# dvl-tum/e-osvos

Hardware: AMD Instinct MI355X
Metric: finetune_iters_per_sec (higher is better)
Workload: dtype f32 (f16x3 split); 1 GPU; e-OSVOS-50 fine-tune iteration (BASELINE configs[1]): DeepLabV3+-ResNet50, batch 3, 480x854, BCE, per-neuron-lr SGD; one (sequence, object) per rank; batch=3, height=480, width=854, parallelism=replicas x1

## Files before the change

### e-osvos_amd/_ffi.py

```python
import ctypes
import os

_HERE = os.path.dirname(os.path.abspath(__file__))
LIB_PATH = os.environ.get('EOSVOS_LIB') or os.path.join(_HERE, 'libeosvos.so')

c_float_p = ctypes.c_void_p
_E = ctypes.c_void_p

_SIGNATURES = {
    'eosvos_version': (ctypes.c_char_p, []),
    'eosvos_last_error': (ctypes.c_char_p, []),
    'eosvos_set_matrix_mode': (ctypes.c_int, [ctypes.c_int]),
    'eosvos_get_matrix_mode': (ctypes.c_int, []),
    'eosvos_set_presplit': (ctypes.c_int, [ctypes.c_int]),
    'eosvos_plan_fingerprint': (ctypes.c_int, [_E, ctypes.POINTER(ctypes.c_uint64)]),
    'eosvos_set_engine_matrix_mode': (ctypes.c_int, [_E, ctypes.c_int]),
    'eosvos_get_engine_matrix_mode': (ctypes.c_int, [_E]),
    'eosvos_set_wg_budget': (ctypes.c_int, [_E, ctypes.c_int]),
    'eosvos_set_side_stream': (ctypes.c_int, [_E, ctypes.c_int]),
    'eosvos_num_convs': (ctypes.c_int, [ctypes.c_int]),
    'eosvos_conv_info': (ctypes.c_int, [ctypes.c_int, ctypes.c_int, ctypes.POINTER(ctypes.c_int64)]),
    'eosvos_param_count': (ctypes.c_int64, [ctypes.c_int]),
    'eosvos_lr_count': (ctypes.c_int64, [ctypes.c_int]),
    'eosvos_norm_count': (ctypes.c_int64, [ctypes.c_int]),
    'eosvos_create': (ctypes.c_int, [ctypes.POINTER(_E), ctypes.c_int, ctypes.c_int, ctypes.c_int,
                                     ctypes.c_int, ctypes.c_int, ctypes.c_int, ctypes.c_void_p]),
    'eosvos_create_ex': (ctypes.c_int, [ctypes.POINTER(_E), ctypes.c_int, ctypes.c_int, ctypes.c_int,
                                        ctypes.c_int, ctypes.c_int, ctypes.c_int, ctypes.c_void_p, ctypes.c_int]),
    'eosvos_destroy': (ctypes.c_int, [_E]),
# ... 123 lines not shown
```

### e-osvos_amd/csrc/conv_kernels.hip

```cpp
#include "kernels.h"

#include <stdlib.h>
#include <string.h>

#include <vector>

namespace eosvos {

typedef float f32x16 __attribute__((ext_vector_type(16)));

#define EOSVOS_BK 32
#define EOSVOS_EB 4
#define EOSVOS_EB128 EOSVOS_EB
#define EOSVOS_OCC 2
#define MFMA32(a, b, c) __builtin_amdgcn_mfma_f32_32x32x2f32((a), (b), (c), 0, 0, 0)

__device__ __forceinline__ int xcd_remap(int bid, int nwg) {
  const int q = nwg >> 3, r = nwg & 7, xcd = bid & 7;
  return (xcd < r ? xcd * (q + 1) : r * (q + 1) + (xcd - r) * q) + (bid >> 3);
}

__device__ __forceinline__ float4 ldg4(const float* p) { return *reinterpret_cast<const float4*>(p); }
__device__ __forceinline__ float4 bufld4(__amdgpu_buffer_rsrc_t r, unsigned byte_off) {
  auto v = __builtin_amdgcn_raw_buffer_load_b128(r, byte_off, 0, 0);
// ... 456 lines not shown
long conv_build_multi_table(const ConvArgs& a, const ConvSegHost* segs, int nseg, std::vector<int>& prefix,
                            std::vector<unsigned char>& taplist, std::vector<ConvTap>& taps) {
  const int chunks = (a.Kc + EOSVOS_BK - 1) / EOSVOS_BK;
  const int nt = (a.N + 127) / 128, mt = (a.M + 127) / 128;
  taps.clear();
  for (int g = 0; g < nseg; ++g) {
    const ConvSegHost& sg = segs[g];
    const int T = sg.k * sg.k;
    for (int ky = 0; ky < sg.k; ++ky)
      for (int kx = 0; kx < sg.k; ++kx) {
        ConvTap t;
        t.dy = sg.pad - ky * sg.dil; t.dx = sg.pad - kx * sg.dil;
        t.xoff = sg.xoff;
        t.wbase = (int)(sg.woff + (long)(ky * sg.k + kx) * a.wK);
        t.wrow = T * a.wK;
        t.ksoff = sg.ksoff; t.seg = g; t.pad_ = 0;
        taps.push_back(t);
      }
  }
  prefix.assign((size_t)mt * nt + 1, 0);
  taplist.assign((size_t)mt * nt * 32, 0);
  long total = 0;
  for (int tm = 0; tm < mt; ++tm) {
    std::vector<unsigned char> keep;
    for (size_t id = 0; id < taps.size(); ++id) {
      bool any = false;
      for (int m = tm * 128; m < a.M && m < tm * 128 + 128 && !any; ++m) {
        const int hw = a.Ho * a.Wo, rem = m % hw;
        const int sy = rem / a.Wo + taps[id].dy, sx = rem % a.Wo + taps[id].dx;
        any = sy >= 0 && sx >= 0 && sy < a.Hi && sx < a.Wi;
      }
// ... 151 lines not shown
            c = MFMA_BF16(fa[tm][0], fb[tn][1], c);
            c = MFMA_BF16(fa[tm][0], fb[tn][0], c);
          } else {
            c = MFMA_F16(__builtin_bit_cast(f16x8, fa[tm][1]), __builtin_bit_cast(f16x8, fb[tn][0]), c);
            c = MFMA_F16(__builtin_bit_cast(f16x8, fa[tm][0]), __builtin_bit_cast(f16x8, fb[tn][1]), c);
            c = MFMA_F16(__builtin_bit_cast(f16x8, fa[tm][0]), __builtin_bit_cast(f16x8, fb[tn][0]), c);
          }
          acc[hm + tm][hn + tn] = c;
        }
    }
  }
}

constexpr int xs_max(int a, int b) { return a > b ? a : b; }
template <int BN, int NP> constexpr int conv_xs_smem() { return xs_max(NP * (128 + BN) * X6_ROWB, 128 * (BN + 4) * 4); }
template <int BN, bool KMAJOR, int NP, bool MULTI = false>
__device__ __forceinline__ void conv_xs_body(const ConvArgs& p, unsigned char* smem) {
  constexpr int BM = 128, BK = 32;
  constexpr int A_BYTES = NP * BM * X6_ROWB;
  constexpr int LDC = BN + 4;
  unsigned char* const As = smem;
  unsigned char* const Bs = smem + A_BYTES;

  const int tid = threadIdx.x, lane = tid & 63, wave = tid >> 6;
  const int wm = wave >> 1, wn = wave & 1;
  const int fr = lane & 15, fq = lane >> 4;

  const int T = p.KH * p.KW;
  const int chunks = (p.Kc + BK - 1) / BK;
  const int ksteps = T * chunks;
  const int nt = (p.N + BN - 1) / BN;
  const int tiles = ((p.M + BM - 1) / BM) * nt;
  const long U = p.tprefix ? (long)p.tprefix[tiles] : (long)tiles * ksteps;
// ... 2 lines not shown
  const long u_begin = sk0 + (long)bid * p.per;
  long u_end = u_begin + p.per;
  if (u_end > U) u_end = U;
  int dp_i = 0;

  constexpr int APASS = BM / 32;
  const int a_c4 = tid & 7, a_r = x6_stage_row(tid);
  constexpr int NQ = BN / 4, RPT = BN / 32;
  constexpr int BPASS = BN / 32;
  const int b_c4 = a_c4, b_r = a_r;
  const int b_n4 = RPT == 4 ? x6_kmaj_c4_128(tid) : x6_kmaj_c4_64(tid);
  const int b_kq = RPT == 4 ? x6_kmaj_kq_128(tid) : x6_kmaj_kq_64(tid);
  const int up = 1 << p.upshift;
  constexpr int TN = BN / 32;
  const __amdgpu_buffer_rsrc_t rx = make_rsrc(p.x, (long)p.B * p.Hi * p.Wi * p.ldx * 4);
  const __amdgpu_buffer_rsrc_t rw = make_rsrc(p.w, MULTI ? p.w_floats * 4 : (p.plane_rows ? (long)p.nplanes : 1L) * p.wN * T * p.wK * 4);
  float sa = 1.f, sb = 1.f, inv_ab = 1.f;
  unsigned h3_ax = 0, h3_ak = 0, h3_aw = 0;
  bool h3_pending = false;
  if (NP == 2 && !MULTI) {
    h3_ax = amax_issue(p.amax_x); h3_ak = amax_issue(KMAJOR ? p.amax_ks : nullptr); h3_aw = amax_issue(p.amax_w);
    h3_pending = true;
  }
  auto scales_late = [&]() {
    if (h3_pending) {
      float ia, ib;
      sa = h3_scale_bits(h3_ax, KMAJOR && p.amax_ks, h3_ak, ia);
      sb = h3_scale_bits(h3_aw, false, 0u, ib);
      inv_ab = ia * ib;
      h3_pending = false;
    }
// ... 81 lines not shown
        a_sx0[i] = ox * p.mul + p.off0;
        a_img[i] = b * p.Hi * p.Wi;
      } else {
        a_sy0[i] = -(1 << 28);
        a_sx0[i] = 0;
        a_img[i] = 0;
      }
    }
    float4 ra[APASS], rb[BPASS];
    constexpr unsigned OOB = 0x80000000u;
    int a_off[APASS];
    int b_off[BPASS];
    const int wplane = p.plane_rows ? (m0 / p.plane_rows) * (int)p.w_plane : 0;
#pragma unroll
    for (int i = 0; i < BPASS; ++i) {
      if (KMAJOR) {
        const int n = n0 + b_n4 * 4;
        b_off[i] = n < p.N ? wplane + (b_kq * RPT + i) * T * p.wK + n : -1;
      } else {
        const int n = n0 + b_r + i * 32;
        b_off[i] = n < p.N ? wplane + n * T * p.wK + b_c4 * 4 : -1;
      }
    }
    int cur_tap = -1;
    int m_wrow = 0, m_ksoff = 0;
    auto load_tiles = [&](int ks) {
      const int vt = ks / chunks;
      const int c0 = (ks - vt * chunks) * BK;
      const int tap = MULTI ? vt : (p.tprefix ? (int)((tappack >> (4 * vt)) & 15) : vt);
      if (tap != cur_tap) {
        cur_tap = tap;
        int dy, dx, xoff = 0;
        if (MULTI) {
          const int id = __builtin_amdgcn_readfirstlane((int)p.taplist[(size_t)tile * 32 + vt]);
          const ConvTap d = p.taps[id];
          dy = d.dy; dx = d.dx; xoff = d.xoff; m_wrow = d.wrow; m_ksoff = d.ksoff; seg_ld = d.seg;
          if (NP == 2) { sa = pick4(seg_sa, seg_ld); sb = pick4(seg_sb, seg_ld); }
#pragma unroll
          for (int i = 0; i < BPASS; ++i) {
            const int n = n0 + b_n4 * 4;
            b_off[i] = n < p.N ? d.wbase + (b_kq * RPT + i) * d.wrow + n : -1;
          }
        } else {
          const int ky = tap / p.KW, kx = tap - ky * p.KW;
          dy = ky * p.kstep; dx = kx * p.kstep;
        }
#pragma unroll
        for (int i = 0; i < APASS; ++i) {
          const int sy = a_sy0[i] + dy, sx = a_sx0[i] + dx;
          bool ok = sy >= 0 && sx >= 0 && ((sy | sx) & (up - 1)) == 0;
          const int iy = sy >> p.upshift, ix = sx >> p.upshift;
          ok = ok && iy < p.Hi && ix < p.Wi;
          a_off[i] = ok ? (a_img[i] + iy * p.Wi + ix) * p.ldx + a_c4 * 4 + xoff : -1;
        }
      }
      const bool cok = (c0 + a_c4 * 4) < p.Kc;
      float4 ks4 = make_float4(1.f, 1.f, 1.f, 1.f);
      if (KMAJOR && p.kscale && cok) ks4 = ldg4(p.kscale + (MULTI ? m_ksoff : 0) + c0 + a_c4 * 4);
#pragma unroll
      for (int i = 0; i < APASS; ++i) {
        const unsigned off = (cok && a_off[i] >= 0) ? (unsigned)(a_off[i] + c0) * 4u : OOB;
        float4 v = bufld4(rx, off);
        if (KMAJOR) { v.x *= ks4.x; v.y *= ks4.y; v.z *= ks4.z; v.w *= ks4.w; }
        ra[i] = v;
      }
#pragma unroll
      for (int i = 0; i < BPASS; ++i) {
        unsigned off;
        if (MULTI) {
          const int k = c0 + b_kq * RPT + i;
          off = (b_off[i] >= 0 && k < p.Kc) ? (unsigned)(b_off[i] + c0 * m_wrow) * 4u : OOB;
        } else if (KMAJOR) {
          const int k = c0 + b_kq * RPT + i;
          off = (b_off[i] >= 0 && k < p.Kc) ? (unsigned)(b_off[i] + (c0 * T + tap) * p.wK) * 4u : OOB;
        } else {
          const int k = c0 + b_c4 * 4;
          off = (b_off[i] >= 0 && k < p.Kc) ? (unsigned)(b_off[i] + tap * p.wK + c0) * 4u : OOB;
        }
        rb[i] = bufld4(rw, off);
      }
    };
    auto store_tiles = [&]() {
#pragma unroll
      for (int i = 0; i < APASS; ++i) {
        uint2 pc[NP];
        xs_split4<NP>(ra[i].x, ra[i].y, ra[i].z, ra[i].w, sa, pc);
#pragma unroll
        for (int q = 0; q < NP; ++q) *reinterpret_cast<uint2*>(As + (q * BM + a_r + i * 32) * X6_ROWB + a_c4 * 8) = pc[q];
      }
      if (!KMAJOR) {
#pragma unroll
        for (int i = 0; i < BPASS; ++i) {
          uint2 pc[NP];
          xs_split4<NP>(rb[i].x, rb[i].y, rb[i].z, rb[i].w, sb, pc);
#pragma unroll
          for (int q = 0; q < NP; ++q) *reinterpret_cast<uint2*>(Bs + (q * BN + b_r + i * 32) * X6_ROWB + b_c4 * 8) = pc[q];
        }
      } else if (RPT == 4) {
#pragma unroll
        for (int j = 0; j < 4; ++j) {
          uint2 pc[NP];
          xs_split4<NP>(f4c(rb[0], j), f4c(rb[1], j), f4c(rb[RPT == 4 ? 2 : 0], j), f4c(rb[RPT == 4 ? 3 : 0], j), sb, pc);
#pragma unroll
          for (int q = 0; q < NP; ++q) *reinterpret_cast<uint2*>(Bs + (q * BN + j * NQ + b_n4) * X6_ROWB + b_kq * 8) = pc[q];
        }
// ... 120 lines not shown
        for (int lr = c_r; lr < BM; lr += CROWS)
          *reinterpret_cast<float4*>(slab + lr * BN + c_c4 * 4) = *reinterpret_cast<const float4*>(Cs + lr * LDC + c_c4 * 4);
      }
    }
    if (!dp) u += ks_end - ks_begin;
  }
  if (NP == 2 && p.amax_y) amax_block_commit(ymax, p.amax_y);
}

template <int BN, bool KMAJOR>
__global__ __launch_bounds__(256, 2) void conv_x6_kernel(const ConvArgs p) {
  __shared__ __attribute__((aligned(16))) unsigned char smem[conv_xs_smem<BN, 3>()];
  conv_xs_body<BN, KMAJOR, 3>(p, smem);
}
#define EOSVOS_H3_OCC64 2
template <int BN, bool KMAJOR>
__global__ __launch_bounds__(256, BN == 64 ? EOSVOS_H3_OCC64 : 2) void conv_h3_kernel(const ConvArgs p) {
  __shared__ __attribute__((aligned(16))) unsigned char smem[conv_xs_smem<BN, 2>()];
  conv_xs_body<BN, KMAJOR, 2>(p, smem);
}
__global__ __launch_bounds__(256, 2) void conv_h3_multi_kernel(const ConvArgs p) {
  __shared__ __attribute__((aligned(16))) unsigned char smem[conv_xs_smem<128, 2>()];
  conv_xs_body<128, true, 2, true>(p, smem);
}
__global__ __launch_bounds__(256, 2) void conv_x6_multi_kernel(const ConvArgs p) {
  __shared__ __attribute__((aligned(16))) unsigned char smem[conv_xs_smem<128, 3>()];
  conv_xs_body<128, true, 3, true>(p, smem);
}

__device__ __forceinline__ void amax_block_commit8(unsigned m, unsigned* slot) {
  __shared__ unsigned wmax8[8];
#pragma unroll
  for (int o = 32; o > 0; o >>= 1) {
    const unsigned t = (unsigned)__shfl_xor((int)m, o);
    m = m > t ? m : t;
  }
  if ((threadIdx.x & 63) == 0) wmax8[threadIdx.x >> 6] = m;
  __syncthreads();
// ... 1031 lines not shown
bool g_prof_on = false;
std::vector<ProfRec> g_prof;
std::vector<hipEvent_t> g_prof_pool;
const char* const kProfNames[] = {
    "conv_x6_kernel<128, false>", "conv_x6_kernel<128, true>", "conv_x6_kernel<64, false>", "conv_x6_kernel<64, true>",
    "wgrad_x6_kernel<128, 128>", "wgrad_x6_kernel<128, 64>", "wgrad_x6_kernel<64, 128>", "wgrad_x6_kernel<64, 64>",
    "conv_igemm_kernel<128, false, *>", "conv_igemm_kernel<128, true, *>", "conv_igemm_kernel<64, false, 0>", "conv_igemm_kernel<64, true, 0>",
    "wgrad_kernel<128, 128>", "wgrad_kernel<128, 64>", "wgrad_kernel<64, 128>", "wgrad_kernel<64, 64>",
    "conv_fixup_kernel",
    "wgrad_x6_group_kernel<128, 128>", "wgrad_x6_group_kernel<128, 64>", "wgrad_x6_group_kernel<64, 128>", "wgrad_x6_group_kernel<64, 64>",
    "conv_h3_kernel<128, false>", "conv_h3_kernel<128, true>", "conv_h3_kernel<64, false>", "conv_h3_kernel<64, true>",
    "wgrad_h3_kernel<128, 128>", "wgrad_h3_kernel<128, 64>", "wgrad_h3_kernel<64, 128>", "wgrad_h3_kernel<64, 64>",
    "wgrad_h3_group_kernel<128, 128>", "wgrad_h3_group_kernel<128, 64>", "wgrad_h3_group_kernel<64, 128>", "wgrad_h3_group_kernel<64, 64>",
    "conv_h3_multi_kernel", "conv_x6_multi_kernel", "conv1x1_stream_kernel<*, 128>", "conv1x1_stream_kernel<*, 64>",
    "conv3x3_stream_kernel",
    "wgrad_p_kernel<256, 256>", "wgrad_p_group_kernel<256, 256>"};
constexpr int kProfKernels = sizeof(kProfNames) / sizeof(kProfNames[0]);
hipEvent_t prof_event() {
  if (!g_prof_pool.empty()) { hipEvent_t e = g_prof_pool.back(); g_prof_pool.pop_back(); return e; }
  hipEvent_t e;
  (void)hipEventCreate(&e);
  return e;
}
struct ProfScope {
  hipStream_t s;
  bool on;
  ProfScope(int kernel, double flops, hipStream_t st) : s(st), on(g_prof_on) {
    if (!on) return;
    ProfRec r{prof_event(), prof_event(), kernel, flops};
    (void)hipEventRecord(r.a, s);
    g_prof.push_back(r);
  }
// ... 109 lines not shown
  {
    constexpr long min_avg = 16, min_chunk = 12, min_fill = 60;
    const bool even_taps = a.total_units <= 0 || a.total_units * 100 >= 85L * tiles * ksteps;
    const long budget = conv_wg_budget(a.wg_budget);
    const long avg = a.total_units > 0 ? a.total_units / tiles : ksteps;
    const long S = tiles > 0 ? budget / tiles : 0;
    if (conv_mfma_mode() == 2 && !a.deep && even_taps && q == 0 && per > 0 && per < avg && S >= 2 && avg >= min_avg && avg / S >= min_chunk &&
        tiles * S * 100 >= min_fill * budget) {
      a.splitk = (int)S; nwg = tiles * S; per = 0;
    }
  }
  a.dp_q = (int)q; a.per = (int)per; a.nwg = (int)nwg;
  return (int)nwg;
}

void launch_conv(ConvArgs& a, hipStream_t s) {
  if (stream3x3_ok(a)) {
    a.dp_q = 0; a.per = 0; a.nwg = 0; a.splitk = 0;
    ProfScope ps(37, 2.0 * a.M * a.N * a.Kc * 9, s);
    launch_stream3x3(a, s);
    return;
  }
  if (const int nc = stream1x1_nc(a)) {
    a.dp_q = 0; a.per = 0; a.nwg = 0; a.splitk = 0;
    ProfScope ps(nc >= 128 ? 35 : 36, 2.0 * a.M * a.N * a.Kc, s);
    if (nc == 128) {
      if (a.Kc == 64) launch_stream1x1<64, 128>(a, s);
      else if (a.Kc == 128) launch_stream1x1<128, 128>(a, s);
      else if (a.Kc == 304) launch_stream1x1<304, 128>(a, s);
      else launch_stream1x1<256, 128>(a, s);
// ... 6 lines not shown
      else if (a.Kc == 304) launch_stream1x1<304, 64>(a, s);
      else launch_stream1x1<512, 64>(a, s);
    }
    return;
  }
  const int bn = conv_bn(a);
  const int nwg = conv_plan(a);
  const long tiles = (long)((a.M + 127) / 128) * ((a.N + bn - 1) / bn);
  const dim3 grid(nwg), block(256);
  const int mode = conv_mfma_mode();
  a.y2_done = (a.y2 && mode == 2) ? 1 : 0;
  const int pk = a.nseg > 0 ? (mode == 2 ? 33 : 34) : (mode == 2 ? 21 : mode == 1 ? 0 : 8) + (bn == 128 ? 0 : 2) + (a.kmajor ? 1 : 0);
  {
  ProfScope ps(pk, 2.0 * a.M * a.N * a.KH * a.KW * a.Kc * conv_exec_frac(a), s);
  if (a.nseg > 0) {
    if (mode == 2) hipLaunchKernelGGL(conv_h3_multi_kernel, grid, block, 0, s, a);
    else hipLaunchKernelGGL(conv_x6_multi_kernel, grid, block, 0, s, a);
  } else if (mode == 2) {
    if (a.kmajor) {
      if (bn == 128) hipLaunchKernelGGL((conv_h3_kernel<128, true>), grid, block, 0, s, a);
      else hipLaunchKernelGGL((conv_h3_kernel<64, true>), grid, block, 0, s, a);
    } else {
      if (bn == 128) hipLaunchKernelGGL((conv_h3_kernel<128, false>), grid, block, 0, s, a);
      else hipLaunchKernelGGL((conv_h3_kernel<64, false>), grid, block, 0, s, a);
    }
  } else if (mode == 1) {
    if (a.kmajor) {
      if (bn == 128) hipLaunchKernelGGL((conv_x6_kernel<128, true>), grid, block, 0, s, a);
      else hipLaunchKernelGGL((conv_x6_kernel<64, true>), grid, block, 0, s, a);
    } else {
      if (bn == 128) hipLaunchKernelGGL((conv_x6_kernel<128, false>), grid, block, 0, s, a);
      else hipLaunchKernelGGL((conv_x6_kernel<64, false>), grid, block, 0, s, a);
    }
  } else if (a.deep == 1) {
    if (a.kmajor) hipLaunchKernelGGL((conv_igemm_kernel<128, true, 1>), grid, block, 0, s, a);
    else hipLaunchKernelGGL((conv_igemm_kernel<128, false, 1>), grid, block, 0, s, a);
// ... 284 lines not shown
```

### e-osvos_amd/csrc/engine.cpp

```cpp
#include <dlfcn.h>
#include <hip/hip_runtime.h>
#include <math.h>
#include <stdio.h>
#include <stdlib.h>
#include <string.h>

#include <algorithm>
#include <cmath>
#include <functional>
#include <map>
#include <set>
#include <string>
#include <vector>

#include "../../include/eosvos.h"
#include "kernels.h"

using namespace eosvos;

static thread_local std::string g_err;
static int fail(const std::string& m) {
  g_err = m;
  return 1;
}
// ... 217 lines not shown
  struct PairBuf {
    unsigned char* p = nullptr;
    float* sc = nullptr;
    int64_t floats = 0;
    bool want = false;
    bool fresh = true;
    bool covered = false;
    long cover_iter = -1;
  };
  std::map<const float*, PairBuf> pairs[2];
  long pair_iter = 0;
  unsigned char* pair_zero = nullptr;
  float* pair_sc_pool = nullptr;
  int pair_sc_used = 0;
  uint64_t plan_fp[2] = {0, 0};
  bool presplit_inflight = false;
  int mode = -1;
  int plan_mode = -1;

  unsigned* amax = nullptr;
  struct AmaxRec { const void* ptr = nullptr; long epoch = -1, zero_epoch = -1; };
  std::vector<AmaxRec> amax_rec;
  long fwd_epoch = 0, bwd_epoch = 0;
  bool w_amax_valid = false;
  long us_zero_epoch = -1;
  long* mt_rbase = nullptr; int* mt_rlen = nullptr; long* mt_toff = nullptr; int2* mt_tit = nullptr; int mt_nent = 0;
  long* amax_w_off = nullptr;
  int* amax_w_n = nullptr;
  std::vector<char> ks_amax_valid;
  struct TRec { int idx; bool valid; };
// ... 31 lines not shown
    allocs.push_back(p);
    return (float*)p;
  }
  float* W_(int ci) { return Wp + t.convs[ci].poff; }
  bool gn() const { return norm_mode == EOSVOS_NORM_GN16; }
  const float* A_(int ci) const { return (t.convs[ci].norm && !gn()) ? na + t.convs[ci].noff : nullptr; }
  const float* G_(int ci) const { return na + t.convs[ci].noff; }
  const float* B_(int ci) const { return t.convs[ci].norm ? nb + t.convs[ci].noff : nullptr; }
};

namespace {

void wino_weights_changed(eosvos_engine* e) {
  for (auto& kv : e->wino_us_valid) kv.second = 0;
  e->w_amax_valid = false;
}

bool trace_on();
enum { AM_X = 0, AM_V = 1, AM_G = 2, AM_DM = 3, AM_W = 4, AM_U = 5, AM_US = 6, AM_KS = 7, AM_KINDS = 8 };
inline size_t amax_col(const eosvos_engine* e, int kind, int ci) {
  const size_t nc = e->t.convs.size(), T = eosvos_engine::TSLOTS;
  if (kind <= AM_V) return (size_t)kind * nc + ci;
  if (kind <= AM_DM) return 2 * nc + T + (size_t)(kind - AM_G) * nc + ci;
  return 4 * nc + 2 * T + (size_t)(kind - AM_W) * nc + ci;
}
inline size_t amax_tcol(const eosvos_engine* e, int phase, int idx) {
  return (phase == 0 ? 2 : 4) * e->t.convs.size() + (size_t)phase * eosvos_engine::TSLOTS + idx;
}
inline void amax_zero(unsigned* first, size_t count, hipStream_t st) { launch_amax_zero(first, (int)count, st); }
inline bool h3_mode() { return conv_mfma_mode() == 2; }
// ... 99 lines not shown
    std::vector<int> n(nc);
    for (size_t ci = 0; ci < nc; ++ci) {
      const ConvL& c = e->t.convs[ci];
      off[ci] = (long)c.poff;
      n[ci] = ((c.cin & 3) || (c.poff & 3)) ? 0 : (int)c.wsize();
    }
    e->amax_w_off = (long*)e->falloc((int64_t)nc * 2);
    e->amax_w_n = (int*)e->falloc((int64_t)nc);
    if (!e->amax_w_off || !e->amax_w_n) return;
    (void)hipMemcpy(e->amax_w_off, off.data(), nc * sizeof(long), hipMemcpyHostToDevice);
    (void)hipMemcpy(e->amax_w_n, n.data(), nc * sizeof(int), hipMemcpyHostToDevice);
  }
  amax_zero(amax_slot(e, AM_W, 0), nc, st);
  launch_absmax_segments(e->Wp, e->amax_w_off, e->amax_w_n, (int)nc, amax_slot(e, AM_W, 0), st);
  e->w_amax_valid = true;
}
const unsigned* amax_ks(eosvos_engine* e, int ci, hipStream_t st) {
  if (amax_init(e) || !e->A_(ci)) return nullptr;
  if (!e->ks_amax_valid[ci]) {
    amax_make(e, AM_KS, ci, e->A_(ci), 1, e->t.convs[ci].cout, e->t.convs[ci].cout, st);
    e->ks_amax_valid[ci] = 1;
  }
  return amax_slot(e, AM_KS, ci);
}
unsigned* amax_wino_weights(eosvos_engine* e, int ci, hipStream_t st) {
  if (!h3_mode() || amax_init(e)) return nullptr;
  unsigned* u = amax_slot(e, AM_U, ci);
  if (e->us_zero_epoch != e->fwd_epoch) {
    amax_zero(u, 1, st);
    amax_zero(amax_slot(e, AM_US, ci), 1, st);
// ... 173 lines not shown
    a.res = res; a.ldres = ldres; a.relu = relu ? 1 : 0;
    if (relu)
      if (uint8_t* m = e->m8w(ykey)) { a.mask8_out = m + (y - ykey) / 4; a.ldm8_out = ldy / 4; }
  }
  attach_tap_table(e, ci, 0, B, a);
  unsigned* gn_yslot = nullptr;
  if (h3_mode() && !amax_init(e)) {
    amax_weights(e, st);
    a.amax_x = tlookup(e, 0, xkey);
    if (!a.amax_x) a.amax_x = amax_get(e, AM_X, ci, x, (long)B * Hi * Wi, c.cin, ldx, st);
    a.amax_w = amax_slot(e, AM_W, ci);
    gn_yslot = twrite_fused(e, 0, ykey, ldy == c.cout);
    if (!gn) a.amax_y = gn_yslot;
  }
  if (!gn && !side) pair_attach(e, 0, ykey, y, ldy == c.cout, a);
  trace("fwd", ci, a.M, a.N, (long)c.T() * c.cin, conv_plan(a), conv_exec_frac(a));
  launch_conv(a, st);
  pair_covered(e, 0, ykey, a);
  if (gn)
    launch_gn_forward(e->zbuf[ci], c.cout, e->G_(ci), e->nb + c.noff, res, ldres, y, ldy, e->gn_stats[ci], e->gn_partial, B,
                      a.Ho * a.Wo, c.cout, 1e-5f, relu ? 1 : 0, st, gn ? gn_yslot : nullptr,
                      (relu && e->m8w(ykey)) ? e->m8w(ykey) + (y - ykey) / 4 : nullptr, ldy / 4);
}
bool dgrad_has_tail(const ConvArgs& a) { return a.N > 128 && a.N % 128 > 0 && a.N % 128 <= 64; }
void launch_dgrad_tail_split(eosvos_engine* e, int ci, ConvArgs a, long K) {
  const int tail = a.N % 128;
  ConvArgs b = a;
  a.N -= tail;
  trace("dgrad", ci, a.M, a.N, K, conv_plan(a));
  launch_conv(a, e->s);
  b.N = tail; b.w += a.N; b.y += a.N;
  if (b.mask8) { b.mask8 += a.N / 4; b.mask_c0 = b.mask_c0 > a.N ? b.mask_c0 - a.N : 0; }
  if (b.res) b.res += a.N;
  trace("dgrad", ci, b.M, b.N, K, conv_plan(b));
  launch_conv(b, e->s);
}
int conv_dgrad(eosvos_engine* e, int ci, const float* g, int ldg, int Hin, int Win, float* gx, int ldgx, int B,
               bool accum, const float* relu_x, int mask_c0, const float* add = nullptr, int ldadd = 0,
               const float* gkey = nullptr, const float* gxkey = nullptr) {
  const uint8_t* mask8 = relu_x ? e->m8(relu_x) : nullptr;
  if (relu_x && !mask8) return fail("internal: a masked data gradient of conv " + std::to_string(ci) + " has no ReLU mask bytes");
  const ConvL& c = e->t.convs[ci];
  ConvArgs a;
// ... 44 lines not shown
    }
    launch_wino_dgrad_output(wg.tm, e->wino_dv, prow, c.cin, B, Hin, Win, th, tw, wg.d, mask8, a.ldm8, mask_c0, accum ? 1 : 0, gx, ldgx, e->s, gxs);
    return 0;
  }
  if (c.k == 1 && c.stride == 2 && !add) {
    if (!accum) (void)hipMemsetAsync(gx, 0, (size_t)B * Hin * Win * ldgx * sizeof(float), e->s);
    a.Ho = a.Hi; a.Wo = a.Wi; a.mul = 1; a.off0 = 0; a.kstep = 0; a.upshift = 0;
    a.M = B * a.Ho * a.Wo; a.dst_up = 1; a.Hf = Hin; a.Wf = Win;
  }
  if (dgrad_has_tail(a) && !a.dst_up && !(c.k == 3 && c.dil >= 2)) {
    launch_dgrad_tail_split(e, ci, a, (long)c.T() * c.cout);
    return 0;
  }
  attach_tap_table(e, ci, 1, B, a);
  pair_attach(e, 1, gxkey, gx, ldgx == c.cin, a);
  trace("dgrad", ci, a.M, a.N, (long)c.T() * c.cout, conv_plan(a), conv_exec_frac(a));
  launch_conv(a, e->s);
  pair_covered(e, 1, gxkey, a);
  return 0;
}
#define EOSVOS_SIDE_BATCH 4
int g_presplit = -1;
bool presplit_switch() {
  if (g_presplit < 0) g_presplit = (getenv("EOSVOS_PRESPLIT") && atoi(getenv("EOSVOS_PRESPLIT")) == 0) ? 0 : 1;
  return g_presplit != 0;
}
bool presplit_enabled(const eosvos_engine* e) {
  return presplit_switch() && h3_mode() && e->force_algo == 0 && (e->s2 || e->presplit_inflight);
}
bool presplit_wgrad_shape(const ConvL& c, int P, int ldg, int ldx) {
// ... 378 lines not shown
  }
  unsigned* amax_w = nullptr;
  if (update) {
    for (auto& kv : e->wino_us_valid)
      if (e->train_from == 0 || kv.first >= lo) kv.second = 0;
    if (h3_mode() && !amax_init(e) && e->w_amax_valid) {
      amax_w = amax_slot(e, AM_W, 0);
      amax_zero(amax_w + lo, (size_t)(hi - lo), stream);
    } else {
      e->w_amax_valid = false;
    }
  }
  launch_sgd_update_all(e->upd_tab[slot], hi - lo, e->upd_blocks[slot], e->Wp, e->ws_wg, e->na,
                        update ? e->lr : nullptr, (update && e->lr_level == EOSVOS_LR_PARAM) ? e->lr_elem : nullptr,
                        accumulate ? e->gsum : nullptr, e->keep_grads ? e->gout : nullptr, stream, amax_w);
  return 0;
}

bool aspp_dgrad_merged(eosvos_engine* e, int B, float* g_l4, const float* l4) {
  const Topo& t = e->t;
  if (e->gn() || !conv_multi_supported() || e->force_algo != 0) return false;
  for (int i = 0; i < 4; ++i) {
    const ConvL& c = t.convs[t.aspp[i]];
    if (c.cout != 256 || c.cin != t.convs[t.aspp[0]].cin || c.stride != 1 || t.aspp[i] != t.aspp[0] + i) return false;
    if (wino_on(e, t.aspp[i], B, e->h16, e->w16)) return false;
  }
  const ConvL& c0 = t.convs[t.aspp[0]];
  ConvArgs a;
  memset(&a, 0, sizeof(a));
  a.wg_budget = e->wg_budget;
// ... 36 lines not shown
    a.amax_x = tlookup(e, 1, e->g_cat);
    if (!a.amax_x) a.amax_x = amax_get(e, AM_G, t.aspp[0], e->g_cat, (long)B * e->h16 * e->w16, 1280, 1280, e->s);
    for (int i = 0; i < 4; ++i) {
      a.seg_amax_w[i] = amax_slot(e, AM_W, t.aspp[i]);
      a.seg_amax_ks[i] = amax_ks(e, t.aspp[i], e->s);
    }
    a.amax_y = twrite_fused(e, 1, g_l4, true);
  }
  double fl = 0;
  for (int i = 0; i < 4; ++i) fl += 2.0 * a.M * a.N * t.convs[t.aspp[i]].T() * 256.0;
  if (trace_on())
    trace_line("dgrad", t.aspp[0], a.M, a.N, (long)(a.total_units * 32 / (((a.M + 127) / 128) * ((a.N + 127) / 128))), conv_plan(a),
               2.0 * 128 * 128 * 32 * (double)a.total_units);
  (void)fl;
  pair_attach(e, 1, g_l4, g_l4, true, a);
  launch_conv(a, e->s);
  pair_covered(e, 1, g_l4, a);
  return true;
}

void plans_match_mode(eosvos_engine* e) {
  const int mode = conv_mfma_mode() | (presplit_switch() ? 16 * g_presplit : 0);
  if (e->plan_mode == mode) return;
  e->plan_mode = mode;
  e->wg_plans.clear();
  for (auto& tab : e->upd_tab) tab = nullptr;
  e->wino_v_batch.clear();
  for (auto& kv : e->wino_dm_batch) kv.second = 0;
}

// ... 10 lines not shown
extern "C" {

const char* eosvos_version(void) { return "eosvos-mi355x 0.8 (gfx950, fp32 implicit GEMM on the fp16 matrix cores: 2-way split, 3 partial products on v_mfma_f32_16x16x32_f16, weight gradients of the stride-16 layers on pre-split fp16-pair operands by LDS-DMA; bf16x6 and fp32-MFMA modes selectable)"; }
const char* eosvos_last_error(void) { return g_err.c_str(); }

int eosvos_set_matrix_mode(int mode) {
  if (mode != EOSVOS_MATRIX_F32 && mode != EOSVOS_MATRIX_BF16X6 && mode != EOSVOS_MATRIX_F16X3) return fail("unknown matrix mode");
  conv_set_mfma_mode(mode);
  return 0;
}
int eosvos_get_matrix_mode(void) { return conv_mfma_mode(); }
int eosvos_plan_fingerprint(eosvos_engine* e, uint64_t* out2) {
  if (!e || !out2) return fail("null argument");
  out2[0] = e->plan_fp[0]; out2[1] = e->plan_fp[1];
  return 0;
}
int eosvos_set_presplit(int on) {
  const int prev = presplit_switch() ? g_presplit : 0;
  g_presplit = on == 2 ? 2 : (on ? 1 : 0);
  return prev;
}
int eosvos_set_engine_matrix_mode(eosvos_engine* e, int mode) {
  if (!e) return fail("null engine");
  if (mode != -1 && mode != EOSVOS_MATRIX_F32 && mode != EOSVOS_MATRIX_BF16X6 && mode != EOSVOS_MATRIX_F16X3) return fail("unknown matrix mode");
  e->mode = mode;
  return 0;
}
int eosvos_get_engine_matrix_mode(eosvos_engine* e) {
  if (!e) { fail("null engine"); return -1; }
  return e->mode >= 0 ? e->mode : conv_mfma_mode();
// ... 1826 lines not shown
```

### e-osvos_amd/csrc/kernels.h

```cpp
#pragma once
#include <hip/hip_runtime.h>
#include <stdint.h>

namespace eosvos {
#define AMAX_SUB 32
#define AMAX_ROW 2048
#if defined(__HIPCC__)
__device__ __forceinline__ unsigned amax_f1(float x) {
  const unsigned a = __float_as_uint(x) & 0x7fffffffu;
  return a < 0x7f800000u ? a : 0u;
}
__device__ __forceinline__ unsigned amax_f4(unsigned m, const float4& v) {
  const unsigned a = amax_f1(v.x), b = amax_f1(v.y), c = amax_f1(v.z), d = amax_f1(v.w);
  const unsigned ab = a > b ? a : b, cd = c > d ? c : d;
  const unsigned q = ab > cd ? ab : cd;
  return m > q ? m : q;
}
__device__ __forceinline__ uint8_t relu_bits(const float4& v) {
  return (uint8_t)((v.x > 0.f ? 1 : 0) | (v.y > 0.f ? 2 : 0) | (v.z > 0.f ? 4 : 0) | (v.w > 0.f ? 8 : 0));
}
__device__ __forceinline__ void relu_mask8(float4& v, unsigned bits) {
  v.x = (bits & 1u) ? v.x : 0.f; v.y = (bits & 2u) ? v.y : 0.f; v.z = (bits & 4u) ? v.z : 0.f; v.w = (bits & 8u) ? v.w : 0.f;
}
__device__ __forceinline__ void amax_block_commit(unsigned m, unsigned* slot) {
// ... 62 lines not shown
  int splitk;
  int wg_budget;
  int nseg;
  const struct ConvTap* taps;
  const unsigned char* taplist;
  long w_floats;
  const unsigned* seg_amax_w[4];
  const unsigned* seg_amax_ks[4];
  const unsigned* amax_x;
  const unsigned* amax_w;
  const unsigned* amax_ks;
  unsigned* amax_y;
  unsigned char* y2;
  const float* y2_sc;
  int y2_done;
};
struct ConvTap {
  int dy, dx;
  int xoff;
  int wbase;
  int wrow;
  int ksoff;
  int seg, pad_;
};
#if defined(__HIPCC__)
__host__ __device__
#endif
inline int conv_par_pixel(int B, int Ho, int Wo, int m) {
  const int He = (Ho + 1) >> 1, Hod = Ho >> 1, We = (Wo + 1) >> 1, Wod = Wo >> 1;
  const int n00 = B * He * We, n01 = B * He * Wod, n10 = B * Hod * We;
  int py, px, r = m;
  if (r < n00) { py = 0; px = 0; }
  else if ((r -= n00) < n01) { py = 0; px = 1; }
  else if ((r -= n01) < n10) { py = 1; px = 0; }
  else { r -= n10; py = 1; px = 1; }
  const int Hc = py ? Hod : He, Wc = px ? Wod : We;
  const int nc = Hc * Wc;
  const int b = r / nc, rr = r - b * nc;
  const int cy = rr / Wc, cx = rr - cy * Wc;
// ... 13 lines not shown
double conv_exec_frac(const struct ConvArgs& a);
double wgrad_exec_frac(const struct WgradArgs& a);
int conv_mfma_mode();
void launch_absmax(const float* x, long rows, int C, int ld, unsigned* slot, hipStream_t s);
void launch_amax_zero(unsigned* first, int count, hipStream_t s);
void launch_absmax_segments(const float* base, const long* dev_off, const int* dev_n, int nseg, unsigned* slots, hipStream_t s);
double launch_mfma_probe(float* scratch, int iters, hipStream_t s);
int64_t conv_ws_floats();
}
#include <vector>
namespace eosvos {
long conv_build_tap_table(const ConvArgs& a, std::vector<int>& prefix, std::vector<int>& mask);
struct ConvSegHost { int k, dil, pad, xoff; long woff; int ksoff; };
long conv_build_multi_table(const ConvArgs& a, const ConvSegHost* segs, int nseg, std::vector<int>& prefix,
                            std::vector<unsigned char>& taplist, std::vector<ConvTap>& taps);
bool conv_multi_supported();

struct WgradArgs {
  const float* g;
  const float* x;
  float* ws;
  int B, Ho, Wo, ldg, Cout;
  int Hi, Wi, ldx, Cin;
  int KH, KW, stride, pad, dil;
  int splits;
  long g_tap_stride, x_tap_stride;
  const unsigned* amax_g;
  const unsigned* amax_x;
  float* scn_g; float* scn_x;
  int margin_g, margin_x;
// ... 178 lines not shown
```

### e-osvos_amd/engine.py

```python
import ctypes

import torch

from . import _ffi
from .topology import ARCH_ID, norm_layers, trainable


def _ptr(t):
    return ctypes.c_void_p(t.data_ptr())


def _optr(t):
    return _ptr(t) if t is not None else None


def _relu_bits(t):
    if t is None:
        return None
    m = (t > 0).to(torch.uint8).reshape(*t.shape[:-1], -1, 4)
    return (m[..., 0] | (m[..., 1] << 1) | (m[..., 2] << 2) | (m[..., 3] << 3)).contiguous()


def _ld(t):
    if t is None:
# ... 18 lines not shown


def check_ignore(ignore):
    v = float(ignore)
    if v != v or v in (float('inf'), float('-inf')) or 0.0 <= v <= 1.0:
        raise ValueError(f'ignore={ignore!r}: the void label must be finite and outside [0, 1]')
    return v


def set_matrix_mode(mode):
    _ffi.check(_ffi.load().eosvos_set_matrix_mode({'f32': 0, 'bf16x6': 1, 'f16x3': 2}[mode]))


def get_matrix_mode():
    return {0: 'f32', 1: 'bf16x6', 2: 'f16x3'}[_ffi.load().eosvos_get_matrix_mode()]


GUARD_ABS_TOL, GUARD_REL_TOL = 1e-4, 1e-4
GUARD_LOSS_REL_TOL, GUARD_STEP_TOL, GUARD_PARAM_TOL, GUARD_FLIP_PIXELS = 1e-4, 5e-3, 1e-6, 4.0
GUARD_LOG = []
_MODE_IDS = {'f32': 0, 'bf16x6': 1, 'f16x3': 2}
_MODE_NAMES = {v: k for k, v in _MODE_IDS.items()}


def _guard_enabled():
    import os
    return os.environ.get('EOSVOS_MODE_GUARD', '1') != '0'


_POOL_WARMED = []
# ... 633 lines not shown
```

### include/eosvos.h

```cpp
#ifndef EOSVOS_H
#define EOSVOS_H

#include <stddef.h>
#include <stdint.h>

#ifdef __cplusplus
extern "C" {
#endif

typedef struct eosvos_engine eosvos_engine;

#define EOSVOS_ARCH_RESNET50 50
#define EOSVOS_ARCH_RESNET101 101
#define EOSVOS_ARCH_V3_RESNET50 1050
#define EOSVOS_ARCH_V3_RESNET101 1101
#define EOSVOS_NORM_BN_FROZEN 0
#define EOSVOS_NORM_GN16 1

const char* eosvos_version(void);
const char* eosvos_last_error(void);

#define EOSVOS_MATRIX_F32 0
#define EOSVOS_MATRIX_BF16X6 1
#define EOSVOS_MATRIX_F16X3 2
int eosvos_set_matrix_mode(int mode);
int eosvos_get_matrix_mode(void);
int eosvos_set_presplit(int on);
int eosvos_plan_fingerprint(eosvos_engine* e, uint64_t* out2);
int eosvos_set_engine_matrix_mode(eosvos_engine* e, int mode);
int eosvos_get_engine_matrix_mode(eosvos_engine* e);

int eosvos_set_wg_budget(eosvos_engine* e, int workgroups);

int eosvos_set_side_stream(eosvos_engine* e, int on);

int eosvos_num_convs(int arch);
int eosvos_conv_info(int arch, int idx, int64_t* info);
int64_t eosvos_param_count(int arch);
int64_t eosvos_lr_count(int arch);
int64_t eosvos_norm_count(int arch);

int eosvos_create(eosvos_engine** out, int arch, int norm_mode, int height, int width,
// ... 145 lines not shown
```

Before: 114.8 finetune_iters/s.

## Pre-split conv weights into f16x3 hi/lo images once per SGD update

Adds a weight-split kernel that converts fp32 weights into scaled f16 hi/lo pairs, in both row-major and K-major layouts, right after each SGD update. Forward and dgrad f16x3 conv kernels, including the multi-segment ASPP kernel, then load the pre-split image instead of splitting weights per tile. This removes repeated per-tile splitting ALU work on every weight load, but adds two weight-sized buffers, an extra kernel per update, and extra tap-table bookkeeping.

```diff
diff --git a/e-osvos_amd/_ffi.py b/e-osvos_amd/_ffi.py
--- a/e-osvos_amd/_ffi.py
+++ b/e-osvos_amd/_ffi.py
@@ -13,6 +13,7 @@
     'eosvos_set_matrix_mode': (ctypes.c_int, [ctypes.c_int]),
     'eosvos_get_matrix_mode': (ctypes.c_int, []),
     'eosvos_set_presplit': (ctypes.c_int, [ctypes.c_int]),
+    'eosvos_set_wsplit': (ctypes.c_int, [ctypes.c_int]),
     'eosvos_plan_fingerprint': (ctypes.c_int, [_E, ctypes.POINTER(ctypes.c_uint64)]),
     'eosvos_set_engine_matrix_mode': (ctypes.c_int, [_E, ctypes.c_int]),
     'eosvos_get_engine_matrix_mode': (ctypes.c_int, [_E]),
diff --git a/e-osvos_amd/csrc/conv_kernels.hip b/e-osvos_amd/csrc/conv_kernels.hip
--- a/e-osvos_amd/csrc/conv_kernels.hip
+++ b/e-osvos_amd/csrc/conv_kernels.hip
@@ -494,7 +494,7 @@
         t.xoff = sg.xoff;
         t.wbase = (int)(sg.woff + (long)(ky * sg.k + kx) * a.wK);
         t.wrow = T * a.wK;
-        t.ksoff = sg.ksoff; t.seg = g; t.pad_ = 0;
+        t.ksoff = sg.ksoff; t.seg = g; t.wbase4 = (int)(sg.woff + 4L * (ky * sg.k + kx) * a.wK);
         taps.push_back(t);
       }
   }
@@ -676,9 +676,10 @@
 
 constexpr int xs_max(int a, int b) { return a > b ? a : b; }
 template <int BN, int NP> constexpr int conv_xs_smem() { return xs_max(NP * (128 + BN) * X6_ROWB, 128 * (BN + 4) * 4); }
-template <int BN, bool KMAJOR, int NP, bool MULTI = false>
+template <int BN, bool KMAJOR, int NP, bool MULTI = false, bool WS = false>
 __device__ __forceinline__ void conv_xs_body(const ConvArgs& p, unsigned char* smem) {
   constexpr int BM = 128, BK = 32;
+  static_assert(!WS || (NP == 2 && (!KMAJOR || BN == 128)), "pre-split weights: f16x3, K-major only 128 wide");
   constexpr int A_BYTES = NP * BM * X6_ROWB;
   constexpr int LDC = BN + 4;
   unsigned char* const As = smem;
@@ -711,7 +712,7 @@
   const int up = 1 << p.upshift;
   constexpr int TN = BN / 32;
   const __amdgpu_buffer_rsrc_t rx = make_rsrc(p.x, (long)p.B * p.Hi * p.Wi * p.ldx * 4);
-  const __amdgpu_buffer_rsrc_t rw = make_rsrc(p.w, MULTI ? p.w_floats * 4 : (p.plane_rows ? (long)p.nplanes : 1L) * p.wN * T * p.wK * 4);
+  const __amdgpu_buffer_rsrc_t rw = make_rsrc(WS ? reinterpret_cast<const float*>(p.wimg) : p.w, MULTI ? p.w_floats * 4 : (p.plane_rows ? (long)p.nplanes : 1L) * p.wN * T * p.wK * 4);
   float sa = 1.f, sb = 1.f, inv_ab = 1.f;
   unsigned h3_ax = 0, h3_ak = 0, h3_aw = 0;
   bool h3_pending = false;
@@ -823,7 +824,10 @@
     const int wplane = p.plane_rows ? (m0 / p.plane_rows) * (int)p.w_plane : 0;
 #pragma unroll
     for (int i = 0; i < BPASS; ++i) {
-      if (KMAJOR) {
+      if (KMAJOR && WS) {
+        const int n = n0 + b_n4 * 4;
+        b_off[i] = n < p.N ? (b_kq * T * p.wK + n + i) * 4 : -1;
+      } else if (KMAJOR) {
         const int n = n0 + b_n4 * 4;
         b_off[i] = n < p.N ? wplane + (b_kq * RPT + i) * T * p.wK + n : -1;
       } else {
@@ -848,7 +852,7 @@
 #pragma unroll
           for (int i = 0; i < BPASS; ++i) {
             const int n = n0 + b_n4 * 4;
-            b_off[i] = n < p.N ? d.wbase + (b_kq * RPT + i) * d.wrow + n : -1;
+            b_off[i] = n >= p.N ? -1 : (WS ? d.wbase4 + (b_kq * d.wrow + n + i) * 4 : d.wbase + (b_kq * RPT + i) * d.wrow + n);
           }
         } else {
           const int ky = tap / p.KW, kx = tap - ky * p.KW;
@@ -877,8 +881,11 @@
       for (int i = 0; i < BPASS; ++i) {
         unsigned off;
         if (MULTI) {
-          const int k = c0 + b_kq * RPT + i;
+          const int k = c0 + b_kq * RPT + (WS ? 0 : i);
           off = (b_off[i] >= 0 && k < p.Kc) ? (unsigned)(b_off[i] + c0 * m_wrow) * 4u : OOB;
+        } else if (KMAJOR && WS) {
+          const int k = c0 + b_kq * RPT;
+          off = (b_off[i] >= 0 && k < p.Kc) ? (unsigned)(b_off[i] + (c0 * T + 4 * tap) * p.wK) * 4u : OOB;
         } else if (KMAJOR) {
           const int k = c0 + b_kq * RPT + i;
           off = (b_off[i] >= 0 && k < p.Kc) ? (unsigned)(b_off[i] + (c0 * T + tap) * p.wK) * 4u : OOB;
@@ -897,7 +904,15 @@
 #pragma unroll
         for (int q = 0; q < NP; ++q) *reinterpret_cast<uint2*>(As + (q * BM + a_r + i * 32) * X6_ROWB + a_c4 * 8) = pc[q];
       }
-      if (!KMAJOR) {
+      if (WS) {
+#pragma unroll
+        for (int i = 0; i < BPASS; ++i) {
+          const uint4 v = __builtin_bit_cast(uint4, rb[i]);
+          unsigned char* const d = KMAJOR ? Bs + (i * NQ + b_n4) * X6_ROWB + b_kq * 8 : Bs + (b_r + i * 32) * X6_ROWB + b_c4 * 8;
+          *reinterpret_cast<uint2*>(d) = make_uint2(v.x, v.y);
+          *reinterpret_cast<uint2*>(d + (NP - 1) * BN * X6_ROWB) = make_uint2(v.z, v.w);
+        }
+      } else if (!KMAJOR) {
 #pragma unroll
         for (int i = 0; i < BPASS; ++i) {
           uint2 pc[NP];
@@ -1048,14 +1063,58 @@
   conv_xs_body<BN, KMAJOR, 3>(p, smem);
 }
 #define EOSVOS_H3_OCC64 2
-template <int BN, bool KMAJOR>
+template <int BN, bool KMAJOR, bool WS = false>
 __global__ __launch_bounds__(256, BN == 64 ? EOSVOS_H3_OCC64 : 2) void conv_h3_kernel(const ConvArgs p) {
   __shared__ __attribute__((aligned(16))) unsigned char smem[conv_xs_smem<BN, 2>()];
-  conv_xs_body<BN, KMAJOR, 2>(p, smem);
-}
+  conv_xs_body<BN, KMAJOR, 2, false, WS>(p, smem);
+}
+template <bool WS = false>
 __global__ __launch_bounds__(256, 2) void conv_h3_multi_kernel(const ConvArgs p) {
   __shared__ __attribute__((aligned(16))) unsigned char smem[conv_xs_smem<128, 2>()];
-  conv_xs_body<128, true, 2, true>(p, smem);
+  conv_xs_body<128, true, 2, true, WS>(p, smem);
+}
+
+__global__ __launch_bounds__(256) void wsplit_kernel(const WsplitEntry* __restrict__ tab, int n, const WsplitEntry one,
+                                                     const float* __restrict__ wp, unsigned char* __restrict__ img_row,
+                                                     unsigned char* __restrict__ img_kmaj, const unsigned* __restrict__ slots) {
+  const int b = (int)blockIdx.x;
+  WsplitEntry en = one;
+  if (tab) {
+    int lo = 0, hi = n - 1;
+    while (lo < hi) {
+      const int mid = (lo + hi + 1) >> 1;
+      if (tab[mid].blk0 <= b) lo = mid; else hi = mid - 1;
+    }
+    en = tab[lo];
+  }
+  float inv;
+  const float s = h3_scale(slots + en.slot, nullptr, inv);
+  const int c4n = en.cin >> 2;
+  const long nblk = (long)(en.cout >> 2) * en.T * c4n;
+  const long idx = (long)(b - en.blk0) * 256 + threadIdx.x;
+  if (idx >= nblk) return;
+  const int c4 = (int)(idx % c4n);
+  const long rest = idx / c4n;
+  const int t = (int)(rest % en.T);
+  const long g = rest / en.T;
+  const long row = (long)en.T * en.cin;
+  const long src = en.w_off + (4 * g * en.T + t) * en.cin + 4 * c4;
+  float4 r[4];
+#pragma unroll
+  for (int i = 0; i < 4; ++i) r[i] = ldg4(wp + src + i * row);
+#pragma unroll
+  for (int i = 0; i < 4; ++i) {
+    uint2 pc[2];
+    xs_split4<2>(r[i].x, r[i].y, r[i].z, r[i].w, s, pc);
+    *reinterpret_cast<uint4*>(img_row + (src + i * row) * 4) = make_uint4(pc[0].x, pc[0].y, pc[1].x, pc[1].y);
+  }
+  unsigned char* const dk = img_kmaj + (en.w_off + ((g * en.T + t) * en.cin + 4 * c4) * 4) * 4;
+#pragma unroll
+  for (int j = 0; j < 4; ++j) {
+    uint2 pc[2];
+    xs_split4<2>(f4c(r[0], j), f4c(r[1], j), f4c(r[2], j), f4c(r[3], j), s, pc);
+    *reinterpret_cast<uint4*>(dk + j * 16) = make_uint4(pc[0].x, pc[0].y, pc[1].x, pc[1].y);
+  }
 }
 __global__ __launch_bounds__(256, 2) void conv_x6_multi_kernel(const ConvArgs p) {
   __shared__ __attribute__((aligned(16))) unsigned char smem[conv_xs_smem<128, 3>()];
@@ -2117,8 +2176,10 @@
     "wgrad_h3_group_kernel<128, 128>", "wgrad_h3_group_kernel<128, 64>", "wgrad_h3_group_kernel<64, 128>", "wgrad_h3_group_kernel<64, 64>",
     "conv_h3_multi_kernel", "conv_x6_multi_kernel", "conv1x1_stream_kernel<*, 128>", "conv1x1_stream_kernel<*, 64>",
     "conv3x3_stream_kernel",
-    "wgrad_p_kernel<256, 256>", "wgrad_p_group_kernel<256, 256>"};
+    "wgrad_p_kernel<256, 256>", "wgrad_p_group_kernel<256, 256>",
+    "wsplit_kernel"};
 constexpr int kProfKernels = sizeof(kProfNames) / sizeof(kProfNames[0]);
+constexpr int kProfWsplit = 40;
 hipEvent_t prof_event() {
   if (!g_prof_pool.empty()) { hipEvent_t e = g_prof_pool.back(); g_prof_pool.pop_back(); return e; }
   hipEvent_t e;
@@ -2258,6 +2319,18 @@
   return (int)nwg;
 }
 
+bool conv_wimg_ok(const ConvArgs& a) {
+  if (conv_mfma_mode() != 2 || a.plane_rows || stream3x3_ok(a) || stream1x1_nc(a)) return false;
+  if ((a.wN & 3) || (a.wK & 3) || (a.N & 3)) return false;
+  return !a.kmajor || conv_bn(a) == 128;
+}
+int wsplit_blocks(int cout, int T, int cin) { return (int)(((long)(cout / 4) * T * (cin / 4) + 255) / 256); }
+void launch_wsplit(const WsplitEntry* dev_tab, int n, int blocks, const WsplitEntry& one, const float* wp, unsigned char* img_row,
+                   unsigned char* img_kmaj, const unsigned* slots, hipStream_t s) {
+  if (blocks < 1) return;
+  ProfScope ps(kProfWsplit, 0.0, s);
+  hipLaunchKernelGGL(wsplit_kernel, dim3(blocks), dim3(256), 0, s, dev_tab, n, one, wp, img_row, img_kmaj, slots);
+}
 void launch_conv(ConvArgs& a, hipStream_t s) {
   if (stream3x3_ok(a)) {
     a.dp_q = 0; a.per = 0; a.nwg = 0; a.splitk = 0;
@@ -2294,12 +2367,17 @@
   {
   ProfScope ps(pk, 2.0 * a.M * a.N * a.KH * a.KW * a.Kc * conv_exec_frac(a), s);
   if (a.nseg > 0) {
-    if (mode == 2) hipLaunchKernelGGL(conv_h3_multi_kernel, grid, block, 0, s, a);
+    if (mode == 2 && a.wimg) hipLaunchKernelGGL(conv_h3_multi_kernel<true>, grid, block, 0, s, a);
+    else if (mode == 2) hipLaunchKernelGGL(conv_h3_multi_kernel<false>, grid, block, 0, s, a);
     else hipLaunchKernelGGL(conv_x6_multi_kernel, grid, block, 0, s, a);
   } else if (mode == 2) {
     if (a.kmajor) {
-      if (bn == 128) hipLaunchKernelGGL((conv_h3_kernel<128, true>), grid, block, 0, s, a);
+      if (bn == 128 && a.wimg) hipLaunchKernelGGL((conv_h3_kernel<128, true, true>), grid, block, 0, s, a);
+      else if (bn == 128) hipLaunchKernelGGL((conv_h3_kernel<128, true>), grid, block, 0, s, a);
       else hipLaunchKernelGGL((conv_h3_kernel<64, true>), grid, block, 0, s, a);
+    } else if (a.wimg) {
+      if (bn == 128) hipLaunchKernelGGL((conv_h3_kernel<128, false, true>), grid, block, 0, s, a);
+      else hipLaunchKernelGGL((conv_h3_kernel<64, false, true>), grid, block, 0, s, a);
     } else {
       if (bn == 128) hipLaunchKernelGGL((conv_h3_kernel<128, false>), grid, block, 0, s, a);
       else hipLaunchKernelGGL((conv_h3_kernel<64, false>), grid, block, 0, s, a);
diff --git a/e-osvos_amd/csrc/engine.cpp b/e-osvos_amd/csrc/engine.cpp
--- a/e-osvos_amd/csrc/engine.cpp
+++ b/e-osvos_amd/csrc/engine.cpp
@@ -255,6 +255,11 @@
   float* pair_sc_pool = nullptr;
   int pair_sc_used = 0;
   uint64_t plan_fp[2] = {0, 0};
+  unsigned char *wimg_row = nullptr, *wimg_kmaj = nullptr;
+  bool wimg_failed = false;
+  std::vector<char> wimg_want, wimg_valid;
+  struct WimgTab { WsplitEntry* dev = nullptr; int lo = -1, hi = -1, n = 0, blocks = 0; bool stale = true; };
+  WimgTab wimg_tab[2];
   bool presplit_inflight = false;
   int mode = -1;
   int plan_mode = -1;
@@ -316,6 +321,7 @@
 void wino_weights_changed(eosvos_engine* e) {
   for (auto& kv : e->wino_us_valid) kv.second = 0;
   e->w_amax_valid = false;
+  std::fill(e->wimg_valid.begin(), e->wimg_valid.end(), 0);
 }
 
 bool trace_on();
@@ -445,6 +451,70 @@
   amax_zero(amax_slot(e, AM_W, 0), nc, st);
   launch_absmax_segments(e->Wp, e->amax_w_off, e->amax_w_n, (int)nc, amax_slot(e, AM_W, 0), st);
   e->w_amax_valid = true;
+  std::fill(e->wimg_valid.begin(), e->wimg_valid.end(), 0);
+}
+
+int g_wsplit = 1;
+WsplitEntry wimg_entry(eosvos_engine* e, int ci, int blk0) {
+  const ConvL& c = e->t.convs[ci];
+  return WsplitEntry{(long)c.poff, c.cout, c.T(), c.cin, (int)amax_col(e, AM_W, ci), blk0, 0};
+}
+bool wimg_init(eosvos_engine* e) {
+  if (e->wimg_row) return true;
+  if (e->wimg_failed) return false;
+  int64_t n = 0;
+  for (const ConvL& c : e->t.convs) n = std::max<int64_t>(n, (int64_t)c.poff + c.wsize());
+  const int64_t keep = e->max_alloc_floats;
+  e->wimg_row = (unsigned char*)e->falloc(n);
+  e->wimg_kmaj = e->wimg_row ? (unsigned char*)e->falloc(n) : nullptr;
+  e->max_alloc_floats = keep;
+  if (!e->wimg_kmaj) {
+    (void)hipGetLastError();
+    e->wimg_row = nullptr;
+    e->wimg_failed = true;
+    return false;
+  }
+  e->wimg_want.assign(e->t.convs.size(), 0);
+  e->wimg_valid.assign(e->t.convs.size(), 0);
+  return true;
+}
+void wimg_attach(eosvos_engine* e, int ci, ConvArgs& a, hipStream_t st, int col = 0) {
+  if (!g_wsplit || !a.amax_w || !e->w_amax_valid || !conv_wimg_ok(a) || !wimg_init(e)) return;
+  const ConvL& c = e->t.convs[ci];
+  if ((c.poff & 3) || (c.cin & 3) || (c.cout & 3)) return;
+  if (!e->wimg_want[ci]) { e->wimg_want[ci] = 1; e->wimg_tab[0].stale = e->wimg_tab[1].stale = true; }
+  if (!e->wimg_valid[ci]) {
+    launch_wsplit(nullptr, 1, wsplit_blocks(c.cout, c.T(), c.cin), wimg_entry(e, ci, 0), e->Wp, e->wimg_row, e->wimg_kmaj, e->amax, st);
+    e->wimg_valid[ci] = 1;
+  }
+  a.wimg = a.kmajor ? e->wimg_kmaj + (size_t)c.poff * 4 + (size_t)col * 16 : e->wimg_row + (size_t)c.poff * 4;
+}
+int wimg_after_update(eosvos_engine* e, int lo, int hi, int part, bool refreshed, hipStream_t stream) {
+  if (!e->wimg_row) return 0;
+  if (!g_wsplit || !refreshed) {
+    std::fill(e->wimg_valid.begin() + lo, e->wimg_valid.begin() + hi, 0);
+    return 0;
+  }
+  auto& tb = e->wimg_tab[part];
+  if (tb.stale || tb.lo != lo || tb.hi != hi) {
+    std::vector<WsplitEntry> tab;
+    int blk = 0;
+    for (int ci = lo; ci < hi; ++ci)
+      if (e->wimg_want[ci]) {
+        tab.push_back(wimg_entry(e, ci, blk));
+        blk += wsplit_blocks(tab.back().cout, tab.back().T, tab.back().cin);
+      }
+    tb.dev = nullptr;
+    if (!tab.empty()) {
+      tb.dev = (WsplitEntry*)e->falloc((int64_t)(tab.size() * sizeof(WsplitEntry) + 3) / 4);
+      if (!tb.dev) return fail("hipMalloc weight-split table");
+      HIPOK(hipMemcpy(tb.dev, tab.data(), tab.size() * sizeof(WsplitEntry), hipMemcpyHostToDevice));
+    }
+    tb.lo = lo; tb.hi = hi; tb.n = (int)tab.size(); tb.blocks = blk; tb.stale = false;
+  }
+  if (tb.n > 0) launch_wsplit(tb.dev, tb.n, tb.blocks, WsplitEntry{}, e->Wp, e->wimg_row, e->wimg_kmaj, e->amax, stream);
+  for (int ci = lo; ci < hi; ++ci) e->wimg_valid[ci] = e->wimg_want[ci];
+  return 0;
 }
 const unsigned* amax_ks(eosvos_engine* e, int ci, hipStream_t st) {
   if (amax_init(e) || !e->A_(ci)) return nullptr;
@@ -648,6 +718,7 @@
     if (!gn) a.amax_y = gn_yslot;
   }
   if (!gn && !side) pair_attach(e, 0, ykey, y, ldy == c.cout, a);
+  wimg_attach(e, ci, a, st);
   trace("fwd", ci, a.M, a.N, (long)c.T() * c.cin, conv_plan(a), conv_exec_frac(a));
   launch_conv(a, st);
   pair_covered(e, 0, ykey, a);
@@ -661,6 +732,7 @@
   const int tail = a.N % 128;
   ConvArgs b = a;
   a.N -= tail;
+  wimg_attach(e, ci, a, e->s);
   trace("dgrad", ci, a.M, a.N, K, conv_plan(a));
   launch_conv(a, e->s);
   b.N = tail; b.w += a.N; b.y += a.N;
@@ -735,6 +807,7 @@
   }
   attach_tap_table(e, ci, 1, B, a);
   pair_attach(e, 1, gxkey, gx, ldgx == c.cin, a);
+  wimg_attach(e, ci, a, e->s);
   trace("dgrad", ci, a.M, a.N, (long)c.T() * c.cout, conv_plan(a), conv_exec_frac(a));
   launch_conv(a, e->s);
   pair_covered(e, 1, gxkey, a);
@@ -1143,6 +1216,7 @@
   launch_sgd_update_all(e->upd_tab[slot], hi - lo, e->upd_blocks[slot], e->Wp, e->ws_wg, e->na,
                         update ? e->lr : nullptr, (update && e->lr_level == EOSVOS_LR_PARAM) ? e->lr_elem : nullptr,
                         accumulate ? e->gsum : nullptr, e->keep_grads ? e->gout : nullptr, stream, amax_w);
+  if (update) return wimg_after_update(e, lo, hi, part, amax_w != nullptr, stream);
   return 0;
 }
 
@@ -1209,6 +1283,12 @@
                2.0 * 128 * 128 * 32 * (double)a.total_units);
   (void)fl;
   pair_attach(e, 1, g_l4, g_l4, true, a);
+  if (h3_mode()) {
+    a.amax_w = a.seg_amax_w[0];
+    for (int i = 0; i < 4; ++i) { a.wimg = nullptr; wimg_attach(e, t.aspp[i], a, e->s); if (!a.wimg) break; }
+    if (a.wimg) a.wimg = e->wimg_kmaj + (size_t)c0.poff * 4;
+    a.amax_w = nullptr;
+  }
   launch_conv(a, e->s);
   pair_covered(e, 1, g_l4, a);
   return true;
@@ -1249,6 +1329,11 @@
   if (!e || !out2) return fail("null argument");
   out2[0] = e->plan_fp[0]; out2[1] = e->plan_fp[1];
   return 0;
+}
+int eosvos_set_wsplit(int on) {
+  const int prev = g_wsplit;
+  g_wsplit = on ? 1 : 0;
+  return prev;
 }
 int eosvos_set_presplit(int on) {
   const int prev = presplit_switch() ? g_presplit : 0;
diff --git a/e-osvos_amd/csrc/kernels.h b/e-osvos_amd/csrc/kernels.h
--- a/e-osvos_amd/csrc/kernels.h
+++ b/e-osvos_amd/csrc/kernels.h
@@ -100,6 +100,7 @@
   unsigned char* y2;
   const float* y2_sc;
   int y2_done;
+  const unsigned char* wimg;
 };
 struct ConvTap {
   int dy, dx;
@@ -107,8 +108,10 @@
   int wbase;
   int wrow;
   int ksoff;
-  int seg, pad_;
-};
+  int seg;
+  int wbase4;
+};
+struct WsplitEntry { long w_off; int cout, T, cin, slot, blk0, pad_; };
 #if defined(__HIPCC__)
 __host__ __device__
 #endif
@@ -152,6 +155,10 @@
 struct ConvSegHost { int k, dil, pad, xoff; long woff; int ksoff; };
 long conv_build_multi_table(const ConvArgs& a, const ConvSegHost* segs, int nseg, std::vector<int>& prefix,
                             std::vector<unsigned char>& taplist, std::vector<ConvTap>& taps);
+bool conv_wimg_ok(const ConvArgs& a);
+int wsplit_blocks(int cout, int T, int cin);
+void launch_wsplit(const WsplitEntry* dev_tab, int n, int blocks, const WsplitEntry& one, const float* wp, unsigned char* img_row,
+                   unsigned char* img_kmaj, const unsigned* slots, hipStream_t s);
 bool conv_multi_supported();
 
 struct WgradArgs {
diff --git a/e-osvos_amd/engine.py b/e-osvos_amd/engine.py
--- a/e-osvos_amd/engine.py
+++ b/e-osvos_amd/engine.py
@@ -56,6 +56,10 @@
 
 def get_matrix_mode():
     return {0: 'f32', 1: 'bf16x6', 2: 'f16x3'}[_ffi.load().eosvos_get_matrix_mode()]
+
+
+def set_wsplit(on):
+    return bool(_ffi.load().eosvos_set_wsplit(1 if on else 0))
 
 
 GUARD_ABS_TOL, GUARD_REL_TOL = 1e-4, 1e-4
diff --git a/include/eosvos.h b/include/eosvos.h
--- a/include/eosvos.h
+++ b/include/eosvos.h
@@ -26,6 +26,7 @@
 int eosvos_set_matrix_mode(int mode);
 int eosvos_get_matrix_mode(void);
 int eosvos_set_presplit(int on);
+int eosvos_set_wsplit(int on);
 int eosvos_plan_fingerprint(eosvos_engine* e, uint64_t* out2);
 int eosvos_set_engine_matrix_mode(eosvos_engine* e, int mode);
 int eosvos_get_engine_matrix_mode(eosvos_engine* e);
```

New measurement: 114.6 finetune_iters/s. About the same (-0.2%).
